# clementinboittiaux/sucre

Measured on AMD Instinct MI355X. Metric: restored Mpixels/sec/GPU at 1080p, 64 neighbour views; % HBM roofline, higher is better.
Workload: dtype f32

## Files before the change

sucre_amd/csrc/experiment.h:

```cpp
#pragma once

#ifdef SUCRE_EXP_NOCOMPUTE
constexpr bool kExpNoCompute = true;
#else
constexpr bool kExpNoCompute = false;
#endif
#ifdef SUCRE_EXP_NOLOAD
constexpr bool kExpNoLoad = true;
#else
constexpr bool kExpNoLoad = false;
#endif
#ifdef SUCRE_EXP_NOSTORE
constexpr bool kExpNoStore = true;
#else
constexpr bool kExpNoStore = false;
#endif
#ifndef SUCRE_STORE_NT
#define SUCRE_STORE_NT 2
#endif
constexpr int kStoreNt = SUCRE_STORE_NT;

#ifndef SUCRE_FIT_WAVES
#define SUCRE_FIT_WAVES 5
#endif
#ifndef SUCRE_CLOSED_WAVES
#define SUCRE_CLOSED_WAVES 4
#endif

#ifndef SUCRE_MIN_STRIPS
#define SUCRE_MIN_STRIPS 4
#endif

#ifndef SUCRE_RING
#define SUCRE_RING 3
#endif
#ifndef SUCRE_DMA_POLICY
#define SUCRE_DMA_POLICY " nt"
#endif

#ifndef SUCRE_EXACT_DIV
#define SUCRE_EXACT_DIV 0
#endif
constexpr bool kExactDiv = SUCRE_EXACT_DIV != 0;

#ifndef SUCRE_EXACT_J_ADAM
#define SUCRE_EXACT_J_ADAM 0
#endif
constexpr bool kExactJAdam = SUCRE_EXACT_J_ADAM != 0;

#if !defined(SUCRE_SCALED_B)
#define SUCRE_SCALED_B 1
#endif
constexpr bool kScaledBBuilt = SUCRE_SCALED_B != 0;

#if !defined(SUCRE_PAIRED_J)
#define SUCRE_PAIRED_J 1
#endif
constexpr bool kPairedBuilt = SUCRE_PAIRED_J != 0;

#if !defined(SUCRE_STAGED_TERMS)
#define SUCRE_STAGED_TERMS 1
#endif
constexpr bool kStagedTerms = SUCRE_STAGED_TERMS != 0;

#ifdef SUCRE_EXP_WAVE_TIMES
constexpr bool kExpWaveTimes = true;
#define SUCRE_EXP_EXPORT extern "C" __attribute__((visibility("default")))
#else
constexpr bool kExpWaveTimes = false;
#define SUCRE_EXP_EXPORT [[maybe_unused]] static
#endif

#ifndef SUCRE_DEAL_FIT
#define SUCRE_DEAL_FIT 64, 50, 38, 28, 20
#endif
#ifndef SUCRE_DEAL_CLOSED
#define SUCRE_DEAL_CLOSED 64, 48, 32, 20
#endif
```

sucre_amd/csrc/match.hip:

```cpp
#include "experiment.h"
#include "launch.h"
#include "match_pixel.h"

namespace sucre {

constexpr int kViewsPerGroup = 16;
#define SUCRE_DPP_STEP(OP, X, CTRL, ROWS, FILL) X = OP(X, (uint32_t)__builtin_amdgcn_update_dpp((int)(FILL), (int)X, CTRL, ROWS, 0xf, false))
__device__ __forceinline__ uint32_t wave_umin_to_last(uint32_t x) {
    SUCRE_DPP_STEP(min, x, 0x111, 0xf, 0xffffffffu); SUCRE_DPP_STEP(min, x, 0x112, 0xf, 0xffffffffu);
    SUCRE_DPP_STEP(min, x, 0x114, 0xf, 0xffffffffu); SUCRE_DPP_STEP(min, x, 0x118, 0xf, 0xffffffffu);
    SUCRE_DPP_STEP(min, x, 0x142, 0xa, 0xffffffffu); SUCRE_DPP_STEP(min, x, 0x143, 0xc, 0xffffffffu);
    return x;
}
__device__ __forceinline__ uint32_t wave_umax_to_last(uint32_t x) {
    SUCRE_DPP_STEP(max, x, 0x111, 0xf, 0u); SUCRE_DPP_STEP(max, x, 0x112, 0xf, 0u);
    SUCRE_DPP_STEP(max, x, 0x114, 0xf, 0u); SUCRE_DPP_STEP(max, x, 0x118, 0xf, 0u);
    SUCRE_DPP_STEP(max, x, 0x142, 0xa, 0u); SUCRE_DPP_STEP(max, x, 0x143, 0xc, 0u);
    return x;
}
#undef SUCRE_DPP_STEP

template <bool kBoth, bool kExt>
__global__ __launch_bounds__(256) __attribute__((amdgpu_waves_per_eu(5, 8))) void match_kernel(uint8_t *__restrict__ obs, uint16_t *__restrict__ cnt,
                                                    const float *__restrict__ depth1, const CamDev c1,
                                                    const sucre_view_t *__restrict__ views, int n_views, int k0,
                                                    int k1, int tiles_x, int n_tiles, int tiles_per_xcd,
                                                    size_t tile_stride, size_t view_stride, uint8_t *__restrict__ ext,
                                                    int ext_mode, uint8_t *__restrict__ ext2,
                                                    uint64_t *__restrict__ vbits, uint2 *__restrict__ zrange) {
    __shared__ __attribute__((aligned(16))) float lz[4][kTilePx];
    __shared__ __attribute__((aligned(16))) uint8_t lc[4][3 * kTilePx];
    __shared__ __attribute__((aligned(16))) float le[kExt ? 4 : 1][kExt ? 3 : 1][kExt ? kTilePx : 1];
    __shared__ __attribute__((aligned(16))) float lf[kBoth ? 4 : 1][kBoth ? 3 : 1][kBoth ? kTilePx : 1];
    const int tile = (blockIdx.x & 7) * tiles_per_xcd + (blockIdx.x >> 3);
    if (tile >= n_tiles) return;
    const int lane = threadIdx.x & 63;
    const int wave = __builtin_amdgcn_readfirstlane(threadIdx.x >> 6);
    const int ty = tile / tiles_x, tx = tile - ty * tiles_x;
    const int u1 = tx * kTile + (lane & 15);
    const int v1b = ty * kTile + (lane >> 4);
    const float W1f = (float)c1.W, H1f = (float)c1.H;
    const bool pin1 = pinhole_form(c1.K) && pinhole_form(c1.Kinv);

    float wP[4][3];
    bool ok1[4];
#pragma unroll
    for (int j = 0; j < 4; ++j) {
        const int v1 = v1b + 4 * j;
        float d = 0.0f;
        if (v1 < c1.H && u1 < c1.W) d = depth1[(size_t)v1 * c1.W + u1];
        ok1[j] = d > 0.0f;
        float cP[3];
        unproject(c1.Kinv, pin1, (float)u1, (float)v1, d, cP);
        rigid(c1.R, c1.t, cP, wP[j]);
    }

    const int kb = k0 + blockIdx.y * kViewsPerGroup;
    const int ke = min(kb + kViewsPerGroup, k1);
    uint32_t zlo = 0xffffffffu, zhi = 0u;
    for (int k = kb + wave; k < ke; k += 4) {
        const sucre_view_t *vw = views + k;
        const uint8_t *__restrict__ rgb2 = vw->rgb;
        const bool packed = rgb2 == nullptr;
        const float W2f = (float)vw->W, H2f = (float)vw->H;
        const bool pin = pin1 && pinhole_form(vw->K) && pinhole_form(vw->Kinv);
        int total = 0;
        unsigned long long bal[4];
#pragma unroll
        for (int j = 0; j < 4; ++j) {
            bool m = ok1[j];
            float z = 0.0f;
            uint32_t r = 0, g = 0, b = 0;
            float c2[3] = {0.f, 0.f, 0.f};
            float f2[3] = {0.f, 0.f, 0.f};
            if (m) {
                size_t q;
                uint32_t rgbw = 0;
                m = match_pixel(c1, W1f, H1f, vw, packed, W2f, H2f, pin, wP[j], u1, v1b + 4 * j, &q, c2, &rgbw);
                if (m) {
                    z = sqrtf(c2[0] * c2[0] + c2[1] * c2[1] + c2[2] * c2[2]);
                    zlo = min(zlo, __float_as_uint(z)); zhi = max(zhi, __float_as_uint(z));
                    if (kBoth) {
                        const auto *pf = global_ptr(reinterpret_cast<const float *>(rgb2)) + q * 3;
                        f2[0] = pf[0]; f2[1] = pf[1]; f2[2] = pf[2];
                    } else if (kExt && ext_mode == SUCRE_EXT_COLOUR) {
                        const auto *pf = global_ptr(reinterpret_cast<const float *>(rgb2)) + q * 3;
                        c2[0] = pf[0]; c2[1] = pf[1]; c2[2] = pf[2];
                    } else {
                        if (!packed) {
                            const bool last = q + 1 == (size_t)vw->H * vw->W;
                            typedef uint32_t __attribute__((aligned(1))) u32_any;
                            rgbw = *(const __attribute__((address_space(1))) u32_any *)(rgb2 + q * 3 - (last ? 1 : 0));
                            rgbw = last ? rgbw >> 8 : rgbw;
                        }
                        r = rgbw & 255u; g = (rgbw >> 8) & 255u; b = (rgbw >> 16) & 255u;
                    }
                }
            }
            const int slot = 64 * j + lane;
            lz[wave][slot] = z;
            lc[wave][slot] = (uint8_t)r; lc[wave][kTilePx + slot] = (uint8_t)g; lc[wave][2 * kTilePx + slot] = (uint8_t)b;
            if constexpr (kExt) { le[wave][0][slot] = m ? c2[0] : 0.f; le[wave][1][slot] = m ? c2[1] : 0.f; le[wave][2][slot] = m ? c2[2] : 0.f; }
            if constexpr (kBoth) { lf[wave][0][slot] = m ? f2[0] : 0.f; lf[wave][1][slot] = m ? f2[1] : 0.f; lf[wave][2][slot] = m ? f2[2] : 0.f; }
            bal[j] = __ballot(m);
            total += __builtin_popcountll(bal[j]);
        }
        if (lane < 4)
            vbits[((size_t)tile * n_views + k) * 4 + lane] = lane == 0 ? bal[0] : lane == 1 ? bal[1] : lane == 2 ? bal[2] : bal[3];
        if (lane == 0) cnt[(size_t)tile * n_views + k] = (uint16_t)total;
        if (k + 4 >= ke) {
            const uint32_t lo = wave_umin_to_last(zlo), hi = wave_umax_to_last(zhi);
            if (lane == 63) zrange[(size_t)tile * n_views + k] = make_uint2(lo, hi);
        } else if (lane == 63) {
            zrange[(size_t)tile * n_views + k] = make_uint2(0xffffffffu, 0u);
        }
        if (total > 0) {
            __builtin_amdgcn_fence(__ATOMIC_RELEASE, "wavefront");
            __builtin_amdgcn_wave_barrier();
            uint8_t *chunk = obs + (size_t)tile * tile_stride + (size_t)k * view_stride;
            *reinterpret_cast<float4 *>(chunk + lane * 16) = *reinterpret_cast<const float4 *>(&lz[wave][lane * 4]);
            uint32_t *c = reinterpret_cast<uint32_t *>(chunk + kChunkZ) + lane;
            const uint32_t *cw = reinterpret_cast<const uint32_t *>(&lc[wave][0]) + lane;
            c[0] = cw[0]; c[64] = cw[64]; c[128] = cw[128];
            if constexpr (kExt) {
                uint8_t *e = ext + ((size_t)tile * n_views + k) * kExtChunk;
#pragma unroll
                for (int pl = 0; pl < 3; ++pl)
                    *reinterpret_cast<float4 *>(e + pl * kChunkZ + lane * 16) = *reinterpret_cast<const float4 *>(&le[wave][pl][lane * 4]);
            }
            if constexpr (kBoth) {
                uint8_t *e = ext2 + ((size_t)tile * n_views + k) * kExtChunk;
#pragma unroll
                for (int pl = 0; pl < 3; ++pl)
                    *reinterpret_cast<float4 *>(e + pl * kChunkZ + lane * 16) = *reinterpret_cast<const float4 *>(&lf[wave][pl][lane * 4]);
            }
            __builtin_amdgcn_fence(__ATOMIC_RELEASE, "wavefront");
            __builtin_amdgcn_wave_barrier();
        }
    }
}

__global__ __launch_bounds__(256) void match_map_kernel(const float *__restrict__ depth1, const CamDev c1,
                                                        const sucre_view_t *__restrict__ views, int k,
                                                        int32_t *__restrict__ map) {
    const int idx = blockIdx.x * 256 + threadIdx.x;
    if (idx >= c1.H * c1.W) return;
    const int v1 = idx / c1.W, u1 = idx - v1 * c1.W;
    const float d = depth1[idx];
    int32_t out = -1;
    if (d > 0.0f) {
        const sucre_view_t *vw = views + k;
        float cP[3], wP[3], c2[3];
        size_t q;
        const bool pin = pinhole_form(c1.K) && pinhole_form(c1.Kinv) && pinhole_form(vw->K) && pinhole_form(vw->Kinv);
        unproject(c1.Kinv, pin, (float)u1, (float)v1, d, cP);
        rigid(c1.R, c1.t, cP, wP);
        uint32_t rgbw;
        if (match_pixel(c1, (float)c1.W, (float)c1.H, vw, vw->rgb == nullptr, (float)vw->W, (float)vw->H, pin, wP, u1, v1, &q, c2, &rgbw))
            out = (int32_t)q;
    }
    map[idx] = out;
}

__global__ __launch_bounds__(256) void project_points_kernel(const CamDev cam, const float *__restrict__ wP, long long n,
                                                             int32_t *__restrict__ pix) {
    const long long i = (long long)blockIdx.x * 256 + threadIdx.x;
    if (i >= n) return;
    const float p[3] = {wP[i], wP[n + i], wP[2 * n + i]};
    float px, py;
    const bool inside = project(cam.Rinv, cam.tinv, cam.K, pinhole_form(cam.K), (float)cam.W, (float)cam.H, p, &px, &py);
    pix[i] = inside ? (int32_t)py * cam.W + (int32_t)px : -1;
}

constexpr int kStatTiles = 32;

__global__ __launch_bounds__(256) void view_partial_kernel(const uint16_t *__restrict__ cnt, int n_tiles, int n_views,
                                                           uint32_t *__restrict__ partial, const uint2 *__restrict__ zrange,
                                                           uint2 *__restrict__ zpart) {
    __shared__ uint32_t plo[4], phi[4];
    const int t0 = blockIdx.x * kStatTiles, n = min(kStatTiles, n_tiles - t0);
    uint32_t zlo = 0xffffffffu, zhi = 0u;
    for (int k = threadIdx.x; k < n_views; k += 256) {
        const uint16_t *p = cnt + (size_t)t0 * n_views + k;
        uint32_t s = 0;
        if (n == kStatTiles) {
#pragma unroll
            for (int i = 0; i < kStatTiles; ++i) s += p[(size_t)i * n_views];
        } else {
            for (int i = 0; i < n; ++i) s += p[(size_t)i * n_views];
        }
        partial[(size_t)blockIdx.x * n_views + k] = s;
    }
    {
        const uint2 *base = zrange + (size_t)t0 * n_views;
        const int total = n * n_views;
        for (int i = threadIdx.x; i < total; i += 256) {
            const uint2 r = base[i];
            zlo = min(zlo, r.x); zhi = max(zhi, r.y);
        }
    }
#pragma unroll
    for (int off = 32; off > 0; off >>= 1) { zlo = min(zlo, (uint32_t)__shfl_xor((int)zlo, off, 64)); zhi = max(zhi, (uint32_t)__shfl_xor((int)zhi, off, 64)); }
    if ((threadIdx.x & 63) == 0) { plo[threadIdx.x >> 6] = zlo; phi[threadIdx.x >> 6] = zhi; }
    __syncthreads();
    if (threadIdx.x == 0) zpart[blockIdx.x] = make_uint2(min(min(plo[0], plo[1]), min(plo[2], plo[3])), max(max(phi[0], phi[1]), max(phi[2], phi[3])));
}

__global__ __launch_bounds__(1024) void view_total_kernel(const uint32_t *__restrict__ partial, int n_rows, int n_views,
                                                          double min_cover, double hw, uint64_t *__restrict__ view_count,
                                                          uint32_t *__restrict__ view_keep, uint64_t *__restrict__ n_obs,
                                                          uint64_t *__restrict__ n_obs_total, const uint2 *__restrict__ zpart,
                                                          uint32_t *__restrict__ zspan) {
    __shared__ unsigned long long part[1024];
    __shared__ unsigned long long wsum[16];
    __shared__ uint32_t plo[16], phi[16];
    const int t = threadIdx.x;
    {
        uint32_t zlo = 0xffffffffu, zhi = 0u;
        for (int i = t; i < n_rows; i += 1024) { const uint2 r = zpart[i]; zlo = min(zlo, r.x); zhi = max(zhi, r.y); }
#pragma unroll
        for (int off = 32; off > 0; off >>= 1) { zlo = min(zlo, (uint32_t)__shfl_xor((int)zlo, off, 64)); zhi = max(zhi, (uint32_t)__shfl_xor((int)zhi, off, 64)); }
        if ((t & 63) == 0) { plo[t >> 6] = zlo; phi[t >> 6] = zhi; }
        __syncthreads();
        if (t == 0) {
            for (int w = 1; w < 16; ++w) { zlo = min(zlo, plo[w]); zhi = max(zhi, phi[w]); }
            zspan[0] = zlo; zspan[1] = zhi;
        }
    }
    int kc = 64;
    while (kc < n_views && kc < 1024) kc <<= 1;
    const int slices = 1024 / kc, k0 = t & (kc - 1), r = t / kc;
    unsigned long long kept = 0;
    for (int kb = 0; kb < n_views; kb += kc) {
        const int k = kb + k0;
        unsigned long long s = 0;
        if (k < n_views) {
            int i = r;
            for (; i + 7 * slices < n_rows; i += 8 * slices) {
                uint32_t v[8];
#pragma unroll
                for (int j = 0; j < 8; ++j) v[j] = partial[(size_t)(i + j * slices) * n_views + k];
#pragma unroll
                for (int j = 0; j < 8; ++j) s += v[j];
            }
            for (; i < n_rows; i += slices) s += partial[(size_t)i * n_views + k];
        }
        part[t] = s;
        __syncthreads();
        if (r == 0 && k < n_views) {
            for (int j = 1; j < slices; ++j) s += part[j * kc + k0];
            const bool keep = (double)s / hw > min_cover;
            view_count[k] = s;
            view_keep[k] = keep ? 1u : 0u;
            if (keep) kept += s;
        }
        __syncthreads();
    }
    for (int off = 32; off > 0; off >>= 1) kept += __shfl_down(kept, off, 64);
    if ((t & 63) == 0) wsum[t >> 6] = kept;
    __syncthreads();
    if (t == 0) {
        unsigned long long total = 0;
        for (int w = 0; w < 16; ++w) total += wsum[w];
        *n_obs = total;
        *n_obs_total = total;
    }
}

__global__ __launch_bounds__(256) void export_view_kernel(const uint8_t *__restrict__ obs,
                                                          const uint16_t *__restrict__ cnt, int n_views, int k,
                                                          int tiles_x, int H, int W, float *__restrict__ z_out,
                                                          uint8_t *__restrict__ rgb_out, size_t tile_stride,
                                                          size_t view_stride) {
    const int tile = blockIdx.x;
    const int slot = threadIdx.x;
    const int ty = tile / tiles_x, tx = tile - ty * tiles_x;
    const int v = ty * kTile + (slot >> 4), u = tx * kTile + (slot & 15);
    if (v >= H || u >= W) return;
    float z = 0.0f;
    uint8_t c[3] = {0, 0, 0};
    if (cnt[(size_t)tile * n_views + k] > 0) {
        const uint8_t *chunk = obs + (size_t)tile * tile_stride + (size_t)k * view_stride;
        z = reinterpret_cast<const float *>(chunk)[slot];
        const uint8_t *p = chunk + kChunkZ + slot;
        c[0] = p[0]; c[1] = p[kTilePx]; c[2] = p[2 * kTilePx];
    }
    const size_t o = (size_t)v * W + u;
    if (z_out) z_out[o] = z;
    if (rgb_out) {
        const bool has = z > 0.0f;
        rgb_out[o * 3 + 0] = has ? c[0] : 0;
        rgb_out[o * 3 + 1] = has ? c[1] : 0;
        rgb_out[o * 3 + 2] = has ? c[2] : 0;
    }
}

__global__ __launch_bounds__(256) void integrity_scan_kernel(const uint8_t *__restrict__ obs,
                                                             const uint16_t *__restrict__ cnt, int n_views, int n_tiles,
                                                             size_t tile_stride, size_t view_stride,
                                                             uint32_t *__restrict__ verdict,
                                                             unsigned long long *__restrict__ positives) {
    const int k = blockIdx.x, slot = threadIdx.x;
    __shared__ unsigned long long s_pos;
    __shared__ uint32_t s_bad;
    if (slot == 0) { s_pos = 0ull; s_bad = 0u; }
    __syncthreads();
    uint32_t bad = 0u, pos = 0u;
    for (int tile = blockIdx.y; tile < n_tiles; tile += gridDim.y) {
        if (cnt[(size_t)tile * n_views + k] == 0) continue;
        const float z = reinterpret_cast<const float *>(obs + (size_t)tile * tile_stride + (size_t)k * view_stride)[slot];
        bad |= (__builtin_isfinite(z) ? 0u : 1u) | (z < 0.0f ? 2u : 0u);
        pos += z > 0.0f ? 1u : 0u;
    }
    if (pos != 0u) atomicAdd(&s_pos, (unsigned long long)pos);
    if (bad != 0u) atomicOr(&s_bad, bad);
    __syncthreads();
    if (slot == 0) {
        if (s_pos != 0ull) atomicAdd(positives + k, s_pos);
        if (s_bad != 0u) atomicOr(verdict + k, s_bad);
    }
}

__global__ void integrity_verdict_kernel(const unsigned long long *__restrict__ positives,
                                         const uint64_t *__restrict__ view_count, int n_views,
                                         uint32_t *__restrict__ verdict) {
    const int k = blockIdx.x * blockDim.x + threadIdx.x;
    if (k < n_views && positives[k] != view_count[k]) verdict[k] |= 4u;
}

__global__ __launch_bounds__(256) void clear_view_kernel(uint8_t *__restrict__ obs, uint16_t *__restrict__ cnt,
                                                         int n_views, int k, size_t tile_stride, size_t view_stride) {
    const int tile = blockIdx.x;
    reinterpret_cast<float *>(obs + (size_t)tile * tile_stride + (size_t)k * view_stride)[threadIdx.x] = 0.0f;
    if (threadIdx.x == 0) cnt[(size_t)tile * n_views + k] = 0;
}

__global__ __launch_bounds__(256) void import_view_kernel(uint8_t *__restrict__ obs, int k, int tiles_x, int H, int W,
                                                          size_t tile_stride, size_t view_stride,
                                                          const int16_t *__restrict__ u1, const int16_t *__restrict__ v1,
                                                          const float *__restrict__ z, const uint8_t *__restrict__ rgb,
                                                          long long n, uint8_t *__restrict__ ext_dense, int n_views,
                                                          const float *__restrict__ ext, uint8_t *__restrict__ ext2_dense) {
    const long long i = (long long)blockIdx.x * 256 + threadIdx.x;
    if (i >= n) return;
    const int u = u1[i], v = v1[i];
    if (u < 0 || v < 0 || u >= W || v >= H) return;
    const int tile = (v / kTile) * tiles_x + (u / kTile);
    const int slot = (v % kTile) * kTile + (u % kTile);
    uint8_t *chunk = obs + (size_t)tile * tile_stride + (size_t)k * view_stride;
    reinterpret_cast<float *>(chunk)[slot] = z[i];
    chunk[kChunkZ + slot] = rgb ? rgb[i * 3 + 0] : (uint8_t)0;
    chunk[kChunkZ + kTilePx + slot] = rgb ? rgb[i * 3 + 1] : (uint8_t)0;
    chunk[kChunkZ + 2 * kTilePx + slot] = rgb ? rgb[i * 3 + 2] : (uint8_t)0;
    if (ext) {
        float *e = reinterpret_cast<float *>(ext_dense + ((size_t)tile * n_views + k) * kExtChunk);
#pragma unroll
        for (int pl = 0; pl < 3; ++pl) e[pl * kTilePx + slot] = ext[(size_t)pl * n + i];
        if (ext2_dense) {
            float *e2 = reinterpret_cast<float *>(ext2_dense + ((size_t)tile * n_views + k) * kExtChunk);
#pragma unroll
            for (int pl = 0; pl < 3; ++pl) e2[pl * kTilePx + slot] = ext[(size_t)(3 + pl) * n + i];
        }
    }
}

__global__ __launch_bounds__(256) void export_view_ext_kernel(const uint8_t *__restrict__ obs, const uint16_t *__restrict__ cnt,
                                                              const uint8_t *__restrict__ ext_dense, int n_views, int k,
                                                              int tiles_x, int H, int W, float *__restrict__ out,
                                                              size_t tile_stride, size_t view_stride) {
    const int tile = blockIdx.x, slot = threadIdx.x;
    const int ty = tile / tiles_x, tx = tile - ty * tiles_x;
    const int v = ty * kTile + (slot >> 4), u = tx * kTile + (slot & 15);
    if (v >= H || u >= W) return;
    float val[3] = {0.f, 0.f, 0.f};
    if (cnt[(size_t)tile * n_views + k] > 0) {
        const float z = reinterpret_cast<const float *>(obs + (size_t)tile * tile_stride + (size_t)k * view_stride)[slot];
        if (z > 0.0f) {
            const float *e = reinterpret_cast<const float *>(ext_dense + ((size_t)tile * n_views + k) * kExtChunk);
#pragma unroll
            for (int pl = 0; pl < 3; ++pl) val[pl] = e[pl * kTilePx + slot];
        }
    }
#pragma unroll
    for (int pl = 0; pl < 3; ++pl) out[((size_t)pl * H + v) * W + u] = val[pl];
}

__global__ __launch_bounds__(256) void count_view_kernel(const uint8_t *__restrict__ obs, uint16_t *__restrict__ cnt,
                                                         int n_views, int k, size_t tile_stride, size_t view_stride,
                                                         uint64_t *__restrict__ vbits, uint2 *__restrict__ zrange) {
    __shared__ int part[4];
    __shared__ uint32_t plo[4], phi[4];
    const int tile = blockIdx.x, t = threadIdx.x;
    const float z = reinterpret_cast<const float *>(obs + (size_t)tile * tile_stride + (size_t)k * view_stride)[t];
    const unsigned long long bal = __ballot(z > 0.0f);
    uint32_t zlo = z > 0.0f ? __float_as_uint(z) : 0xffffffffu, zhi = z > 0.0f ? __float_as_uint(z) : 0u;
#pragma unroll
    for (int off = 32; off > 0; off >>= 1) { zlo = min(zlo, (uint32_t)__shfl_xor((int)zlo, off, 64)); zhi = max(zhi, (uint32_t)__shfl_xor((int)zhi, off, 64)); }
    if ((t & 63) == 0) {
        vbits[((size_t)tile * n_views + k) * 4 + (t >> 6)] = bal;
        part[t >> 6] = __builtin_popcountll(bal);
        plo[t >> 6] = zlo; phi[t >> 6] = zhi;
    }
    __syncthreads();
    if (t == 0) {
        cnt[(size_t)tile * n_views + k] = (uint16_t)(part[0] + part[1] + part[2] + part[3]);
        zrange[(size_t)tile * n_views + k] = make_uint2(min(min(plo[0], plo[1]), min(plo[2], plo[3])), max(max(phi[0], phi[1]), max(phi[2], phi[3])));
    }
}

hipError_t launch_export_view_ext(const Layout &L, const uint8_t *ws, const uint8_t *ext_dense, int k, float *out, hipStream_t s) {
    hipLaunchKernelGGL(export_view_ext_kernel, dim3(L.n_tiles), dim3(256), 0, s, ws + L.off_obs,
                       reinterpret_cast<const uint16_t *>(ws + L.off_cnt), ext_dense, L.n_views, k, L.tiles_x, L.H, L.W, out,
                       L.obs_tile_stride, L.obs_view_stride);
    return hipGetLastError();
}

hipError_t launch_import_view(const Layout &L, uint8_t *ws, int k, const int16_t *u1, const int16_t *v1, const float *z,
                              const uint8_t *rgb, long long n, hipStream_t s, uint8_t *ext_dense, const float *ext,
                              uint8_t *ext2_dense) {
    auto *cnt = reinterpret_cast<uint16_t *>(ws + L.off_cnt);
    hipLaunchKernelGGL(clear_view_kernel, dim3(L.n_tiles), dim3(256), 0, s, ws + L.off_obs, cnt, L.n_views, k,
                       L.obs_tile_stride, L.obs_view_stride);
    if (n > 0)
        hipLaunchKernelGGL(import_view_kernel, dim3((unsigned)((n + 255) / 256)), dim3(256), 0, s, ws + L.off_obs, k,
                           L.tiles_x, L.H, L.W, L.obs_tile_stride, L.obs_view_stride, u1, v1, z, rgb, n, ext_dense, L.n_views, ext, ext2_dense);
    hipLaunchKernelGGL(count_view_kernel, dim3(L.n_tiles), dim3(256), 0, s, ws + L.off_obs, cnt, L.n_views, k,
                       L.obs_tile_stride, L.obs_view_stride, reinterpret_cast<uint64_t *>(ws + L.off_vbits),
                       reinterpret_cast<uint2 *>(ws + L.off_zrange));
    return hipGetLastError();
}

template <bool kAligned>
__global__ __launch_bounds__(256) void pack_view_kernel(const float *__restrict__ depth, const uint8_t *__restrict__ rgb,
                                                        long long n, uint2 *__restrict__ out) {
    const long long q = (long long)blockIdx.x * 256 + threadIdx.x, i = q * 4;
    if (i >= n) return;
    if (kAligned && i + 4 <= n) {
        const float4 d = *reinterpret_cast<const float4 *>(depth + i);
        const uint32_t *c = reinterpret_cast<const uint32_t *>(rgb + i * 3);
        const uint32_t c0 = c[0], c1 = c[1], c2 = c[2];
        uint4 *o = reinterpret_cast<uint4 *>(out + i);
        o[0] = make_uint4(__float_as_uint(d.x), c0 & 0xffffffu, __float_as_uint(d.y), (c0 >> 24) | ((c1 & 0xffffu) << 8));
        o[1] = make_uint4(__float_as_uint(d.z), (c1 >> 16) | ((c2 & 0xffu) << 16), __float_as_uint(d.w), c2 >> 8);
        return;
    }
    for (long long j = i; j < n && j < i + 4; ++j) {
        const uint8_t *p = rgb + j * 3;
        out[j] = make_uint2(__float_as_uint(depth[j]), (uint32_t)p[0] | ((uint32_t)p[1] << 8) | ((uint32_t)p[2] << 16));
    }
}

constexpr int kPackBatch = 16;
struct PackBatch { const float *depth[kPackBatch]; const uint8_t *rgb[kPackBatch]; uint2 *out[kPackBatch]; };

__global__ __launch_bounds__(256) void pack_views_kernel(const PackBatch b, long long n) {
    const float *__restrict__ depth = b.depth[blockIdx.y];
    const uint8_t *__restrict__ rgb = b.rgb[blockIdx.y];
    uint2 *__restrict__ out = b.out[blockIdx.y];
    const long long q = (long long)blockIdx.x * 256 + threadIdx.x, i = q * 4;
    if (i >= n) return;
    const bool al = reinterpret_cast<uintptr_t>(depth) % 16 == 0 && reinterpret_cast<uintptr_t>(rgb) % 4 == 0 && reinterpret_cast<uintptr_t>(out) % 16 == 0;
    if (al && i + 4 <= n) {
        const float4 d = *reinterpret_cast<const float4 *>(depth + i);
        const uint32_t *c = reinterpret_cast<const uint32_t *>(rgb + i * 3);
        const uint32_t c0 = c[0], c1 = c[1], c2 = c[2];
        uint4 *o = reinterpret_cast<uint4 *>(out + i);
        o[0] = make_uint4(__float_as_uint(d.x), c0 & 0xffffffu, __float_as_uint(d.y), (c0 >> 24) | ((c1 & 0xffffu) << 8));
        o[1] = make_uint4(__float_as_uint(d.z), (c1 >> 16) | ((c2 & 0xffu) << 16), __float_as_uint(d.w), c2 >> 8);
        return;
    }
    for (long long j = i; j < n && j < i + 4; ++j) {
        const uint8_t *p = rgb + j * 3;
        out[j] = make_uint2(__float_as_uint(depth[j]), (uint32_t)p[0] | ((uint32_t)p[1] << 8) | ((uint32_t)p[2] << 16));
    }
}

hipError_t launch_pack_views(const float *const *depth, const uint8_t *const *rgb, void *const *packed, int n, int H, int W, hipStream_t s) {
    const long long px = (long long)H * W, threads = (px + 3) / 4;
    for (int k0 = 0; k0 < n; k0 += kPackBatch) {
        PackBatch b;
        const int m = n - k0 < kPackBatch ? n - k0 : kPackBatch;
        for (int j = 0; j < kPackBatch; ++j) {
            const int k = k0 + (j < m ? j : 0);
            b.depth[j] = depth[k]; b.rgb[j] = rgb[k]; b.out[j] = static_cast<uint2 *>(packed[k]);
        }
        hipLaunchKernelGGL(pack_views_kernel, dim3((unsigned)((threads + 255) / 256), (unsigned)m), dim3(256), 0, s, b, px);
    }
    return hipGetLastError();
}

hipError_t launch_pack_view(const float *depth, const uint8_t *rgb, int H, int W, void *packed, hipStream_t s) {
    const long long n = (long long)H * W, threads = (n + 3) / 4;
    const bool aligned = reinterpret_cast<uintptr_t>(depth) % 16 == 0 && reinterpret_cast<uintptr_t>(rgb) % 4 == 0 && reinterpret_cast<uintptr_t>(packed) % 16 == 0;
    if (aligned) hipLaunchKernelGGL(pack_view_kernel<true>, dim3((unsigned)((threads + 255) / 256)), dim3(256), 0, s, depth, rgb, n, static_cast<uint2 *>(packed));
    else hipLaunchKernelGGL(pack_view_kernel<false>, dim3((unsigned)((threads + 255) / 256)), dim3(256), 0, s, depth, rgb, n, static_cast<uint2 *>(packed));
    return hipGetLastError();
}

hipError_t launch_project_points(const sucre_view_t &view, const float *wP, long long n, int32_t *pix, hipStream_t s) {
    if (n > 0)
        hipLaunchKernelGGL(project_points_kernel, dim3((unsigned)((n + 255) / 256)), dim3(256), 0, s, to_cam(view), wP, n, pix);
    return hipGetLastError();
}

hipError_t launch_match(const Layout &L, uint8_t *ws, const sucre_view_t &target, const sucre_view_t *views_dev,
                        int k0, int k1, hipStream_t s, uint8_t *ext, int ext_mode, uint8_t *ext2) {
    const int tiles_per_xcd = (L.n_tiles + 7) / 8;
    const dim3 grid(8 * tiles_per_xcd, (k1 - k0 + kViewsPerGroup - 1) / kViewsPerGroup);
    auto *cnt = reinterpret_cast<uint16_t *>(ws + L.off_cnt);
    auto *vbits = reinterpret_cast<uint64_t *>(ws + L.off_vbits);
    auto launch = [&](auto kernel, int mode) {
        hipLaunchKernelGGL(kernel, grid, dim3(256), 0, s, ws + L.off_obs, cnt, target.depth, to_cam(target), views_dev, L.n_views, k0,
                           k1, L.tiles_x, L.n_tiles, tiles_per_xcd, L.obs_tile_stride, L.obs_view_stride, ext, mode, ext2, vbits,
                           reinterpret_cast<uint2 *>(ws + L.off_zrange));
    };
    if (ext2) launch(match_kernel<true, true>, SUCRE_EXT_POINTS_COLOUR);
    else if (ext) launch(match_kernel<false, true>, ext_mode);
    else launch(match_kernel<false, false>, ext_mode);
    return hipGetLastError();
}

hipError_t launch_match_map(const Layout &L, const sucre_view_t &target, const sucre_view_t *views_dev, int k,
                            int32_t *map, hipStream_t s) {
    hipLaunchKernelGGL(match_map_kernel, dim3((L.H * L.W + 255) / 256), dim3(256), 0, s, target.depth, to_cam(target),
                       views_dev, k, map);
    return hipGetLastError();
}

hipError_t launch_finalize(const Layout &L, uint8_t *ws, double min_cover, hipStream_t s, const uint8_t *ext_dense,
                           uint8_t *ext_comp, int fmt, const uint8_t *ext2_dense, uint8_t *ext2_comp) {
    auto *cnt = reinterpret_cast<const uint16_t *>(ws + L.off_cnt);
    auto *vc = reinterpret_cast<uint64_t *>(ws + L.off_view_count);
    auto *vk = reinterpret_cast<uint32_t *>(ws + L.off_view_keep);
    auto *partial = reinterpret_cast<uint32_t *>(ws + L.off_view_partial);
    const int rows = (L.n_tiles + kStatTiles - 1) / kStatTiles;
    auto *zpart = reinterpret_cast<uint2 *>(ws + L.off_zpart);
    hipLaunchKernelGGL(view_partial_kernel, dim3(rows), dim3(256), 0, s, cnt, L.n_tiles, L.n_views, partial,
                       reinterpret_cast<const uint2 *>(ws + L.off_zrange), zpart);
    hipLaunchKernelGGL(view_total_kernel, dim3(1), dim3(1024), 0, s, partial, rows, L.n_views, min_cover,
                       (double)L.W * (double)L.H, vc, vk, reinterpret_cast<uint64_t *>(ws + L.off_n_obs),
                       reinterpret_cast<uint64_t *>(ws + L.off_n_obs_total), zpart,
                       reinterpret_cast<uint32_t *>(ws + off_range_span(L)));
    if (hipError_t e = hipGetLastError(); e != hipSuccess) return e;
    return launch_compact(L, ws, s, ext_dense, ext_comp, fmt, ext2_dense, ext2_comp);
}

hipError_t launch_check_store(const Layout &L, const uint8_t *ws, uint32_t *verdict, uint64_t *scratch, hipStream_t s) {
    if (hipError_t e = hipMemsetAsync(verdict, 0, sizeof(uint32_t) * L.n_views, s); e != hipSuccess) return e;
    if (hipError_t e = hipMemsetAsync(scratch, 0, sizeof(uint64_t) * L.n_views, s); e != hipSuccess) return e;
    int per_view = 4096 / L.n_views;
    per_view = per_view < 1 ? 1 : (per_view > L.n_tiles ? L.n_tiles : per_view);
    hipLaunchKernelGGL(integrity_scan_kernel, dim3(L.n_views, per_view), dim3(256), 0, s, ws + L.off_obs,
                       reinterpret_cast<const uint16_t *>(ws + L.off_cnt), L.n_views, L.n_tiles, L.obs_tile_stride,
                       L.obs_view_stride, verdict, reinterpret_cast<unsigned long long *>(scratch));
    hipLaunchKernelGGL(integrity_verdict_kernel, dim3((L.n_views + 255) / 256), dim3(256), 0, s,
                       reinterpret_cast<const unsigned long long *>(scratch),
                       reinterpret_cast<const uint64_t *>(ws + L.off_view_count), L.n_views, verdict);
    return hipGetLastError();
}

hipError_t launch_export_view(const Layout &L, const uint8_t *ws, int k, float *z, uint8_t *rgb, hipStream_t s) {
    hipLaunchKernelGGL(export_view_kernel, dim3(L.n_tiles), dim3(256), 0, s, ws + L.off_obs,
                       reinterpret_cast<const uint16_t *>(ws + L.off_cnt), L.n_views, k, L.tiles_x, L.H, L.W, z, rgb,
                       L.obs_tile_stride, L.obs_view_stride);
    return hipGetLastError();
}

}
```

sucre_amd/csrc/match_pixel.h:

```cpp
#pragma once
#include "experiment.h"
#include "launch.h"

namespace sucre {

__device__ __forceinline__ float dot3(const float *a, float x, float y, float z) {
    float acc = a[0] * x;
    acc = __builtin_fmaf(a[1], y, acc);
    acc = __builtin_fmaf(a[2], z, acc);
    return acc;
}

__host__ __device__ __forceinline__ bool pinhole_form(const float *M) {
    return M[1] == 0.f && M[3] == 0.f && M[6] == 0.f && M[7] == 0.f && M[8] == 1.f;
}

__device__ __forceinline__ void mul3(const float *M, bool pin, float x, float y, float z, float out[3]) {
    if (pin) {
        out[0] = __builtin_fmaf(M[2], z, M[0] * x);
        out[1] = __builtin_fmaf(M[5], z, M[4] * y);
        out[2] = z;
    } else {
        out[0] = dot3(M + 0, x, y, z);
        out[1] = dot3(M + 3, x, y, z);
        out[2] = dot3(M + 6, x, y, z);
    }
}

__device__ __forceinline__ void unproject(const float *Kinv, bool pin, float u, float v, float d, float out[3]) {
    const float x = d * (u + 0.5f), y = d * (v + 0.5f), z = d * 1.0f;
    mul3(Kinv, pin, x, y, z, out);
}

__device__ __forceinline__ void rigid(const float *R, const float *t, const float p[3], float out[3]) {
    out[0] = dot3(R + 0, p[0], p[1], p[2]) + t[0];
    out[1] = dot3(R + 3, p[0], p[1], p[2]) + t[1];
    out[2] = dot3(R + 6, p[0], p[1], p[2]) + t[2];
}

__device__ __forceinline__ void pixel_quotients(float x, float y, float z, float *px, float *py) {
    if (kExactDiv) {
        *px = x / z;
        *py = y / z;
        return;
    }
    const float rc = __builtin_amdgcn_rcpf(z);
    float ax = x * rc, ay = y * rc;
    const float sx = __builtin_fmaf(-__builtin_fabsf(ax), 0x1p-21f, __builtin_fabsf(ax - __builtin_rintf(ax)));
    const float sy = __builtin_fmaf(-__builtin_fabsf(ay), 0x1p-21f, __builtin_fabsf(ay - __builtin_rintf(ay)));
    const bool unsure = !(sx > 0x1p-23f) || !(sy > 0x1p-23f);
    if (__builtin_amdgcn_ballot_w64(unsure) != 0ull) {
        ax = x / z;
        ay = y / z;
    }
    *px = ax;
    *py = ay;
}

__device__ __forceinline__ bool project(const float *Rinv, const float *tinv, const float *K, bool pin, float Wf, float Hf,
                                        const float wP[3], float *px, float *py) {
    float cP[3], c[3];
    rigid(Rinv, tinv, wP, cP);
    mul3(K, pin, cP[0], cP[1], cP[2], c);
    pixel_quotients(c[0], c[1], c[2], px, py);
    return (*px > -1.0f) && (*px < Wf) && (*py > -1.0f) && (*py < Hf);
}

template <class T>
__device__ __forceinline__ const __attribute__((address_space(1))) T *global_ptr(const T *p) {
    return (const __attribute__((address_space(1))) T *)p;
}

__device__ __forceinline__ bool match_pixel(const CamDev &c1, float W1f, float H1f, const sucre_view_t *vw, bool packed,
                                            float W2f, float H2f, bool pin, const float wP[3], int u1, int v1,
                                            size_t *q_out, float c2[3], uint32_t *rgbw) {
    float px, py;
    if (!project(vw->Rinv, vw->tinv, vw->K, pin, W2f, H2f, wP, &px, &py)) return false;
    const int u2 = (int)px, v2 = (int)py;
    const size_t q = (size_t)v2 * vw->W + u2;
    float d2;
    if (packed) {
        const unsigned long long rec = global_ptr(reinterpret_cast<const unsigned long long *>(vw->depth))[q];
        d2 = __uint_as_float((uint32_t)rec);
        *rgbw = (uint32_t)(rec >> 32);
    } else {
        d2 = global_ptr(vw->depth)[q];
    }
    if (!(d2 > 0.0f)) return false;
    float w2[3], qx, qy;
    unproject(vw->Kinv, pin, (float)u2, (float)v2, d2, c2);
    rigid(vw->R, vw->t, c2, w2);
    if (!project(c1.Rinv, c1.tinv, c1.K, pin, W1f, H1f, w2, &qx, &qy)) return false;
    if ((int)qx != u1 || (int)qy != v1) return false;
    *q_out = q;
    return true;
}

inline CamDev to_cam(const sucre_view_t &v) {
    CamDev c;
    for (int i = 0; i < 9; ++i) { c.K[i] = v.K[i]; c.Kinv[i] = v.Kinv[i]; c.R[i] = v.R[i]; c.Rinv[i] = v.Rinv[i]; }
    for (int i = 0; i < 3; ++i) { c.t[i] = v.t[i]; c.tinv[i] = v.tinv[i]; }
    c.H = v.H; c.W = v.W;
    return c;
}

}
```

Measured before the change: 88.85.

## Overlap gather loads of two pixels and speculatively fetch colour in match

Splits match_pixel into land/landing_depth/close stages and processes two pixels per round, issuing both depth gathers (and, for unpacked views, a speculative colour gather) before a single vmcnt wait. The goal is more memory-level parallelism per wave and avoiding a serialized dependent colour load after the depth check. In exchange it adds register pressure and issues colour loads for pixels that may fail the consistency check, which costs extra bandwidth.

```diff
diff --git a/sucre_amd/csrc/experiment.h b/sucre_amd/csrc/experiment.h
--- a/sucre_amd/csrc/experiment.h
+++ b/sucre_amd/csrc/experiment.h
@@ -63,6 +63,16 @@
 #endif
 constexpr bool kStagedTerms = SUCRE_STAGED_TERMS != 0;
 
+#if !defined(SUCRE_MATCH_ROUNDS)
+#define SUCRE_MATCH_ROUNDS 2
+#endif
+#if !defined(SUCRE_MATCH_SPECULATE)
+#define SUCRE_MATCH_SPECULATE (SUCRE_MATCH_ROUNDS == 2)
+#endif
+static_assert(SUCRE_MATCH_ROUNDS == 1 || SUCRE_MATCH_ROUNDS == 2, "SUCRE_MATCH_ROUNDS is 1 or 2");
+constexpr int kMatchInFlight = SUCRE_MATCH_ROUNDS == 2 ? 2 : 1;
+constexpr bool kMatchSpeculate = SUCRE_MATCH_SPECULATE != 0;
+
 #ifdef SUCRE_EXP_WAVE_TIMES
 constexpr bool kExpWaveTimes = true;
 #define SUCRE_EXP_EXPORT extern "C" __attribute__((visibility("default")))
diff --git a/sucre_amd/csrc/match.hip b/sucre_amd/csrc/match.hip
--- a/sucre_amd/csrc/match.hip
+++ b/sucre_amd/csrc/match.hip
@@ -5,6 +5,7 @@
 namespace sucre {
 
 constexpr int kViewsPerGroup = 16;
+constexpr int kWaitVm0 = 0x0f70;
 #define SUCRE_DPP_STEP(OP, X, CTRL, ROWS, FILL) X = OP(X, (uint32_t)__builtin_amdgcn_update_dpp((int)(FILL), (int)X, CTRL, ROWS, 0xf, false))
 __device__ __forceinline__ uint32_t wave_umin_to_last(uint32_t x) {
     SUCRE_DPP_STEP(min, x, 0x111, 0xf, 0xffffffffu); SUCRE_DPP_STEP(min, x, 0x112, 0xf, 0xffffffffu);
@@ -66,44 +67,121 @@
         const bool pin = pin1 && pinhole_form(vw->K) && pinhole_form(vw->Kinv);
         int total = 0;
         unsigned long long bal[4];
-#pragma unroll
-        for (int j = 0; j < 4; ++j) {
-            bool m = ok1[j];
-            float z = 0.0f;
-            uint32_t r = 0, g = 0, b = 0;
-            float c2[3] = {0.f, 0.f, 0.f};
-            float f2[3] = {0.f, 0.f, 0.f};
-            if (m) {
-                size_t q;
-                uint32_t rgbw = 0;
-                m = match_pixel(c1, W1f, H1f, vw, packed, W2f, H2f, pin, wP[j], u1, v1b + 4 * j, &q, c2, &rgbw);
+        constexpr int P = kMatchInFlight;
+        constexpr bool kSpec = kMatchSpeculate && !kExt;
+        if constexpr (P == 1 && !kSpec) {
+#pragma unroll
+            for (int j = 0; j < 4; ++j) {
+                bool m = ok1[j];
+                float z = 0.0f;
+                uint32_t r = 0, g = 0, b = 0;
+                float c2[3] = {0.f, 0.f, 0.f};
+                float f2[3] = {0.f, 0.f, 0.f};
                 if (m) {
-                    z = sqrtf(c2[0] * c2[0] + c2[1] * c2[1] + c2[2] * c2[2]);
-                    zlo = min(zlo, __float_as_uint(z)); zhi = max(zhi, __float_as_uint(z));
-                    if (kBoth) {
-                        const auto *pf = global_ptr(reinterpret_cast<const float *>(rgb2)) + q * 3;
-                        f2[0] = pf[0]; f2[1] = pf[1]; f2[2] = pf[2];
-                    } else if (kExt && ext_mode == SUCRE_EXT_COLOUR) {
-                        const auto *pf = global_ptr(reinterpret_cast<const float *>(rgb2)) + q * 3;
-                        c2[0] = pf[0]; c2[1] = pf[1]; c2[2] = pf[2];
-                    } else {
-                        if (!packed) {
-                            const bool last = q + 1 == (size_t)vw->H * vw->W;
-                            typedef uint32_t __attribute__((aligned(1))) u32_any;
-                            rgbw = *(const __attribute__((address_space(1))) u32_any *)(rgb2 + q * 3 - (last ? 1 : 0));
-                            rgbw = last ? rgbw >> 8 : rgbw;
+                    size_t q;
+                    uint32_t rgbw = 0;
+                    m = match_pixel(c1, W1f, H1f, vw, packed, W2f, H2f, pin, wP[j], u1, v1b + 4 * j, &q, c2, &rgbw);
+                    if (m) {
+                        z = sqrtf(c2[0] * c2[0] + c2[1] * c2[1] + c2[2] * c2[2]);
+                        zlo = min(zlo, __float_as_uint(z)); zhi = max(zhi, __float_as_uint(z));
+                        if (kBoth) {
+                            const auto *pf = global_ptr(reinterpret_cast<const float *>(rgb2)) + q * 3;
+                            f2[0] = pf[0]; f2[1] = pf[1]; f2[2] = pf[2];
+                        } else if (kExt && ext_mode == SUCRE_EXT_COLOUR) {
+                            const auto *pf = global_ptr(reinterpret_cast<const float *>(rgb2)) + q * 3;
+                            c2[0] = pf[0]; c2[1] = pf[1]; c2[2] = pf[2];
+                        } else {
+                            if (!packed) {
+                                const bool last = q + 1 == (size_t)vw->H * vw->W;
+                                rgbw = colour_word(landing_colour(rgb2, q, last), last);
+                            }
+                            r = rgbw & 255u; g = (rgbw >> 8) & 255u; b = (rgbw >> 16) & 255u;
                         }
-                        r = rgbw & 255u; g = (rgbw >> 8) & 255u; b = (rgbw >> 16) & 255u;
                     }
                 }
+                const int slot = 64 * j + lane;
+                lz[wave][slot] = z;
+                lc[wave][slot] = (uint8_t)r; lc[wave][kTilePx + slot] = (uint8_t)g; lc[wave][2 * kTilePx + slot] = (uint8_t)b;
+                if constexpr (kExt) { le[wave][0][slot] = m ? c2[0] : 0.f; le[wave][1][slot] = m ? c2[1] : 0.f; le[wave][2][slot] = m ? c2[2] : 0.f; }
+                if constexpr (kBoth) { lf[wave][0][slot] = m ? f2[0] : 0.f; lf[wave][1][slot] = m ? f2[1] : 0.f; lf[wave][2][slot] = m ? f2[2] : 0.f; }
+                bal[j] = __ballot(m);
+                total += __builtin_popcountll(bal[j]);
             }
-            const int slot = 64 * j + lane;
-            lz[wave][slot] = z;
-            lc[wave][slot] = (uint8_t)r; lc[wave][kTilePx + slot] = (uint8_t)g; lc[wave][2 * kTilePx + slot] = (uint8_t)b;
-            if constexpr (kExt) { le[wave][0][slot] = m ? c2[0] : 0.f; le[wave][1][slot] = m ? c2[1] : 0.f; le[wave][2][slot] = m ? c2[2] : 0.f; }
-            if constexpr (kBoth) { lf[wave][0][slot] = m ? f2[0] : 0.f; lf[wave][1][slot] = m ? f2[1] : 0.f; lf[wave][2][slot] = m ? f2[2] : 0.f; }
-            bal[j] = __ballot(m);
-            total += __builtin_popcountll(bal[j]);
+        } else {
+            auto put = [&](int j, bool m, float z, uint32_t r, uint32_t g, uint32_t b, const float *c2, const float *f2) __attribute__((always_inline)) {
+                const int slot = 64 * j + lane;
+                lz[wave][slot] = z;
+                lc[wave][slot] = (uint8_t)r; lc[wave][kTilePx + slot] = (uint8_t)g; lc[wave][2 * kTilePx + slot] = (uint8_t)b;
+                if constexpr (kExt) { le[wave][0][slot] = m ? c2[0] : 0.f; le[wave][1][slot] = m ? c2[1] : 0.f; le[wave][2][slot] = m ? c2[2] : 0.f; }
+                if constexpr (kBoth) { lf[wave][0][slot] = m ? f2[0] : 0.f; lf[wave][1][slot] = m ? f2[1] : 0.f; lf[wave][2][slot] = m ? f2[2] : 0.f; }
+                bal[j] = __ballot(m);
+                total += __builtin_popcountll(bal[j]);
+            };
+            auto observe = [&](size_t q, bool early, bool last, uint32_t rgbw, float *c2, float *f2, float *z, uint32_t *r, uint32_t *g, uint32_t *b) __attribute__((always_inline)) {
+                *z = sqrtf(c2[0] * c2[0] + c2[1] * c2[1] + c2[2] * c2[2]);
+                zlo = min(zlo, __float_as_uint(*z)); zhi = max(zhi, __float_as_uint(*z));
+                if (kBoth) {
+                    const auto *pf = global_ptr(reinterpret_cast<const float *>(rgb2)) + q * 3;
+                    f2[0] = pf[0]; f2[1] = pf[1]; f2[2] = pf[2];
+                } else if (kExt && ext_mode == SUCRE_EXT_COLOUR) {
+                    const auto *pf = global_ptr(reinterpret_cast<const float *>(rgb2)) + q * 3;
+                    c2[0] = pf[0]; c2[1] = pf[1]; c2[2] = pf[2];
+                } else {
+                    if (!packed) {
+                        if (!early) {
+                            last = q + 1 == (size_t)vw->H * vw->W;
+                            rgbw = landing_colour(rgb2, q, last);
+                        }
+                        rgbw = colour_word(rgbw, last);
+                    }
+                    *r = rgbw & 255u; *g = (rgbw >> 8) & 255u; *b = (rgbw >> 16) & 255u;
+                }
+            };
+#pragma unroll
+            for (int j0 = 0; j0 < 4; j0 += P) {
+                bool m[P], last[P];
+                int u2[P], v2[P];
+                size_t ql[P], q[P];
+                float d2[P], z[P];
+                uint32_t rgbw[P], r[P], g[P], b[P];
+                float c2[P][3], f2[P][3];
+#pragma unroll
+                for (int p = 0; p < P; ++p) {
+                    m[p] = ok1[j0 + p];
+                    u2[p] = 0; v2[p] = 0; ql[p] = 0; q[p] = 0;
+                    d2[p] = 0.0f; rgbw[p] = 0; last[p] = false;
+                    if (m[p]) m[p] = land(vw, W2f, H2f, pin, wP[j0 + p], &u2[p], &v2[p], &ql[p]);
+                }
+                if (packed) {
+#pragma unroll
+                    for (int p = 0; p < P; ++p)
+                        if (m[p]) d2[p] = landing_depth(vw, true, ql[p], &rgbw[p]);
+                } else {
+#pragma unroll
+                    for (int p = 0; p < P; ++p)
+                        if (m[p]) {
+                            d2[p] = landing_depth(vw, false, ql[p], &rgbw[p]);
+                            if (kSpec) {
+                                last[p] = ql[p] + 1 == (size_t)vw->H * vw->W;
+                                rgbw[p] = landing_colour(rgb2, ql[p], last[p]);
+                            }
+                        }
+                }
+                __builtin_amdgcn_s_waitcnt(kWaitVm0);
+#pragma unroll
+                for (int p = 0; p < P; ++p) {
+                    c2[p][0] = 0.f; c2[p][1] = 0.f; c2[p][2] = 0.f;
+                    if (m[p]) m[p] = close(c1, W1f, H1f, vw, pin, u2[p], v2[p], ql[p], d2[p], u1, v1b + 4 * (j0 + p), &q[p], c2[p]);
+                }
+#pragma unroll
+                for (int p = 0; p < P; ++p) {
+                    z[p] = 0.0f; r[p] = 0; g[p] = 0; b[p] = 0;
+                    f2[p][0] = 0.f; f2[p][1] = 0.f; f2[p][2] = 0.f;
+                    if (m[p]) observe(q[p], kSpec, last[p], rgbw[p], c2[p], f2[p], &z[p], &r[p], &g[p], &b[p]);
+                }
+#pragma unroll
+                for (int p = 0; p < P; ++p) put(j0 + p, m[p], z[p], r[p], g[p], b[p], c2[p], f2[p]);
+            }
         }
         if (lane < 4)
             vbits[((size_t)tile * n_views + k) * 4 + lane] = lane == 0 ? bal[0] : lane == 1 ? bal[1] : lane == 2 ? bal[2] : bal[3];
diff --git a/sucre_amd/csrc/match_pixel.h b/sucre_amd/csrc/match_pixel.h
--- a/sucre_amd/csrc/match_pixel.h
+++ b/sucre_amd/csrc/match_pixel.h
@@ -71,21 +71,32 @@
     return (const __attribute__((address_space(1))) T *)p;
 }
 
-__device__ __forceinline__ bool match_pixel(const CamDev &c1, float W1f, float H1f, const sucre_view_t *vw, bool packed,
-                                            float W2f, float H2f, bool pin, const float wP[3], int u1, int v1,
-                                            size_t *q_out, float c2[3], uint32_t *rgbw) {
+__device__ __forceinline__ bool land(const sucre_view_t *vw, float W2f, float H2f, bool pin, const float wP[3], int *u2, int *v2,
+                                     size_t *q) {
     float px, py;
     if (!project(vw->Rinv, vw->tinv, vw->K, pin, W2f, H2f, wP, &px, &py)) return false;
-    const int u2 = (int)px, v2 = (int)py;
-    const size_t q = (size_t)v2 * vw->W + u2;
-    float d2;
+    *u2 = (int)px; *v2 = (int)py;
+    *q = (size_t)*v2 * vw->W + *u2;
+    return true;
+}
+
+__device__ __forceinline__ float landing_depth(const sucre_view_t *vw, bool packed, size_t q, uint32_t *rgbw) {
     if (packed) {
         const unsigned long long rec = global_ptr(reinterpret_cast<const unsigned long long *>(vw->depth))[q];
-        d2 = __uint_as_float((uint32_t)rec);
         *rgbw = (uint32_t)(rec >> 32);
-    } else {
-        d2 = global_ptr(vw->depth)[q];
+        return __uint_as_float((uint32_t)rec);
     }
+    return global_ptr(vw->depth)[q];
+}
+
+__device__ __forceinline__ uint32_t landing_colour(const uint8_t *rgb2, size_t q, bool last) {
+    typedef uint32_t __attribute__((aligned(1))) u32_any;
+    return *(const __attribute__((address_space(1))) u32_any *)(rgb2 + q * 3 - (last ? 1 : 0));
+}
+__device__ __forceinline__ uint32_t colour_word(uint32_t gathered, bool last) { return last ? gathered >> 8 : gathered; }
+
+__device__ __forceinline__ bool close(const CamDev &c1, float W1f, float H1f, const sucre_view_t *vw, bool pin, int u2, int v2,
+                                      size_t q, float d2, int u1, int v1, size_t *q_out, float c2[3]) {
     if (!(d2 > 0.0f)) return false;
     float w2[3], qx, qy;
     unproject(vw->Kinv, pin, (float)u2, (float)v2, d2, c2);
@@ -94,6 +105,16 @@
     if ((int)qx != u1 || (int)qy != v1) return false;
     *q_out = q;
     return true;
+}
+
+__device__ __forceinline__ bool match_pixel(const CamDev &c1, float W1f, float H1f, const sucre_view_t *vw, bool packed,
+                                            float W2f, float H2f, bool pin, const float wP[3], int u1, int v1,
+                                            size_t *q_out, float c2[3], uint32_t *rgbw) {
+    int u2, v2;
+    size_t q;
+    if (!land(vw, W2f, H2f, pin, wP, &u2, &v2, &q)) return false;
+    const float d2 = landing_depth(vw, packed, q, rgbw);
+    return close(c1, W1f, H1f, vw, pin, u2, v2, q, d2, u1, v1, q_out, c2);
 }
 
 inline CamDev to_cam(const sucre_view_t &v) {
```

Result: no change. 89.35, median of 6 (+0.6%).
